# ipilter/RayTracerTest

Hardware: AMD Instinct MI355X
Metric: Mray/s at 1920x1080x16spp (higher is better)
Workload: dtype f32

## Files before the change

### include/rt_mi355x.h

```cpp
#ifndef RT_MI355X_H
#define RT_MI355X_H

#include <stddef.h>
#include <stdint.h>

#ifdef __cplusplus
extern "C" {
#endif

#define RT_OK              0
#define RT_ERR_INVALID     1
#define RT_ERR_NO_DEVICE   2
#define RT_ERR_HIP         3
#define RT_ERR_STATE       4

#define RT_MATH_FMA        0u
#define RT_MATH_STRICT     1u

#define RT_FLAG_NO_FILTER  1u
#define RT_FLAG_NO_BINNING 2u

#define RT_FLAG_NEAREST_HIT 4u

#define RT_FLAG_NO_MACRO_BINS 16u
// ... 153 lines not shown
int  rt_tracer_set_band(rt_tracer* t, uint32_t row_begin, uint32_t rows);
int  rt_tracer_gather_time(rt_tracer* t, double* total_ms, uint64_t* gathers, int reset_after);
int  rt_tracer_gather_only(rt_tracer* t);
int  rt_tracer_group_info(rt_tracer* t, char* json, size_t capacity);
int  rt_tracer_band_count(rt_tracer* t);
int  rt_tracer_band_info(rt_tracer* t, uint32_t band, uint32_t out[4]);

int rt_dbg_hit_triangle(int device, uint32_t math_mode, uint32_t n, const float* rays,
                        const float* tris, int eps_mode, int32_t* hit, float* tuv, float* normal,
                        float* point);
int rt_dbg_sincos(int device, uint32_t n, const float* x, float* s, float* c);
int rt_dbg_trace_occupancy(int device, int samples_in_flight, uint32_t lds_bytes);
int rt_dbg_valu_peak(int device, double* lane_fma_per_s, double* clock_ghz);
int rt_dbg_check_midrange(int device, uint64_t out[4]);
int rt_dbg_wave_list_counts(rt_tracer* t, int half, uint32_t* dst, size_t capacity_tiles, uint32_t* n_tiles, uint32_t* capacity_per_tile);
int rt_dbg_read_tile_lists(rt_tracer* t, uint32_t* dst, size_t capacity_words, uint32_t* words_per_tile);
int rt_dbg_focal_boxes(rt_tracer* t, float curv_scale, float* boxes, size_t boxes_capacity, float* focal, size_t focal_capacity);
int rt_dbg_classify(rt_tracer* t, uint32_t level, uint32_t forms, uint32_t slack_milli, const uint32_t* regions, uint32_t n_regions,
                    float* out, size_t capacity_floats);
int rt_dbg_bvh_build(const rt_float4* rows, size_t count, int edges_layout, void* nodes, size_t node_capacity_bytes,
                     void* leaf_records, size_t leaf_capacity_bytes, uint64_t info[8]);
int rt_dbg_feature_normals(const rt_float4* rows, size_t count, int edges_layout, void* out, size_t capacity_bytes, uint64_t info[8]);
int rt_dbg_exposure_rays(rt_tracer* t, const float* points, size_t n, const float* dirs, uint32_t n_dirs, uint32_t flags,
                         float* segs_out);
int rt_dbg_bvh_refit(const rt_float4* rows, size_t count, int edges_layout, void* nodes, size_t node_bytes, void* leaf_records,
                     size_t record_bytes, uint64_t info[8]);
double rt_dbg_bvh_tree_cost(const void* nodes, size_t node_bytes);
int rt_dbg_query_tree_read(rt_tracer* t, void* nodes, size_t node_capacity_bytes, void* records, size_t record_capacity_bytes,
                           uint64_t info[8]);
int rt_dbg_query_accel_slack(rt_tracer* t, uint32_t slack_milli);
int rt_dbg_query_stack_cap(rt_tracer* t, uint32_t cap);
int rt_dbg_uniform(int device, uint32_t n, uint32_t m, uint32_t* states, float* out);
int rt_dbg_get_ray(rt_tracer* t, uint32_t n, const uint32_t* pixels, uint32_t* states, float* rays);
void rt_dbg_rng_init_host(uint64_t seed, uint64_t subsequence, uint32_t state[6]);
void rt_dbg_rng_advance_host(uint32_t state[5], uint32_t n, int use_table);
void rt_dbg_rng_advance_host_n(uint32_t* states, uint32_t count, uint32_t n, int use_table);
int rt_dbg_owed_state(rt_tracer* t, uint64_t out[4]);
int rt_dbg_enqueue_calls(rt_tracer* t, uint64_t out[8]);

#ifdef __cplusplus
}
#endif
#endif
```

### raytracertest_amd/api.py

```python
import ctypes as C
import os
import threading
import weakref

import numpy as np

_HERE = os.path.dirname(os.path.abspath(__file__))
_LIB_PATH = os.environ.get("RT_MI355X_LIB") or os.path.join(_HERE, "lib", "librt_mi355x.so")

MATH_FMA, MATH_STRICT = 0, 1
FLAG_NO_FILTER = 1
FLAG_NO_BINNING = 2
FLAG_NEAREST_HIT = 4
FLAG_SMOOTH_NORMALS = 8
FLAG_NO_MACRO_BINS = 16
FLAG_NO_SUPER_BINS = 64
FLAG_NO_SURE_HIT = 32
BUF_RENDER, BUF_COUNTS, BUF_IMAGE, BUF_RNG, BUF_FRAME = 0, 1, 2, 3, 4
GROUP_ID_BYTES = 128
TRANSPORT_RCCL, TRANSPORT_PEER = 0, 1

ABI_SYMBOLS = [
    "rt_tracer_create", "rt_tracer_create_ex", "rt_tracer_destroy", "rt_tracer_trace",
    "rt_tracer_stop", "rt_tracer_resize", "rt_tracer_set_camera_parameters",
    "rt_tracer_rotate_camera", "rt_tracer_upload_scene", "rt_tracer_set_update_callback",
    "rt_tracer_set_finished_callback", "rt_tracer_wait", "rt_tracer_set_seed",
    "rt_tracer_upload_spheres", "rt_tracer_trace_enqueue", "rt_tracer_trace_enqueue_n", "rt_tracer_sync", "rt_tracer_trace_stats", "rt_tracer_launch", "rt_tracer_launch_iterations", "rt_tracer_fused_iterations", "rt_tracer_set_image_mirror", "rt_tracer_set_list_reuse", "rt_tracer_stream_b", "rt_tracer_upload_scene_edges", "rt_pack_normal",
    "rt_unpack_normal",
    "rt_tracer_kernel_time", "rt_tracer_launch_time", "rt_tracer_read_buffer", "rt_tracer_copy_buffer_to_device", "rt_tracer_copy_buffer_to_device_async",
    "rt_tracer_stream",
    "rt_tracer_device_pointer", "rt_tracer_buffer_bytes", "rt_tracer_info",
    "rt_tracer_last_error", "rt_last_error", "rt_device_count", "rt_version",
    "rt_dbg_hit_triangle", "rt_dbg_sincos", "rt_dbg_valu_peak", "rt_dbg_check_midrange", "rt_dbg_trace_occupancy", "rt_dbg_uniform", "rt_dbg_get_ray",
    "rt_dbg_rng_init_host", "rt_dbg_rng_advance_host", "rt_dbg_rng_advance_host_n", "rt_dbg_owed_state", "rt_dbg_enqueue_calls",
    "rt_tracer_create_multi", "rt_group_unique_id", "rt_tracer_join_group", "rt_tracer_leave_group",
    "rt_tracer_gather_time", "rt_tracer_band_count", "rt_tracer_band_info",
    "rt_tracer_join_group_bands", "rt_balance_rows", "rt_tracer_rebalance", "rt_tracer_set_band", "rt_dbg_read_tile_lists", "rt_dbg_wave_list_counts", "rt_dbg_focal_boxes", "rt_dbg_classify",
    "rt_tracer_gather_only", "rt_tracer_group_info",
    "rt_tracer_intersect", "rt_tracer_intersect_device", "rt_tracer_pick", "rt_tracer_focus_at",
    "rt_tracer_occluded", "rt_tracer_occluded_device",
    "rt_tracer_exposure", "rt_tracer_exposure_device", "rt_dbg_exposure_rays",
    "rt_tracer_intersect_all", "rt_tracer_intersect_all_device",
    "rt_tracer_closest_point", "rt_tracer_closest_point_device",
    "rt_tracer_closest_all", "rt_tracer_closest_all_device",
    "rt_tracer_signed_distance", "rt_tracer_signed_distance_device",
    "rt_tracer_closest_sides", "rt_tracer_closest_sides_device", "rt_dbg_feature_normals",
    "rt_tracer_overlap", "rt_tracer_overlap_device",
    "rt_tracer_set_query_accel", "rt_tracer_query_accel_info", "rt_dbg_bvh_build", "rt_dbg_query_accel_slack",
    "rt_tracer_set_query_accel_update", "rt_tracer_query_accel_rebuild", "rt_tracer_query_accel_update_info",
    "rt_dbg_bvh_refit", "rt_dbg_query_tree_read", "rt_dbg_bvh_tree_cost", "rt_dbg_query_stack_cap",
]


class RtError(RuntimeError):
    pass


PRIM_NONE = -1
RT_MAX_HITS = 16
RT_MAX_DIRS = 64
EXPOSURE_LOCAL, EXPOSURE_WORLD = 0, 1
QUERY_SCAN, QUERY_BVH = 0, 1
ACCEL_REBUILD, ACCEL_REFIT = 0, 1
BVH_NODE_DTYPE = np.dtype([("lo", np.float32, (3, 4)), ("hi", np.float32, (3, 4)), ("child", np.uint32, 4), ("cmax", np.float32, 4)])
BVH_RECORD_DTYPE = np.dtype([("e2", np.float32, 3), ("e1", np.float32, 3), ("v0", np.float32, 3), ("index", np.uint32), ("pad", np.uint32, 2)])
BVH_EMPTY, BVH_LEAF = 0xFFFFFFFF, 0x80000000
_ACCEL_KEYS = ("mode", "valid", "nodes", "leaves", "depth", "always_tested", "build_us", "device_bytes")
# ... 185 lines not shown
        L.rt_tracer_copy_buffer_to_device.argtypes = [vp, C.c_int, vp, C.c_size_t]
        L.rt_tracer_copy_buffer_to_device_async.argtypes = [vp, C.c_int, vp, C.c_size_t]
        L.rt_tracer_stream.argtypes = [vp]
        L.rt_tracer_stream.restype = vp
        L.rt_tracer_stream_b.argtypes = [vp]
        L.rt_tracer_stream_b.restype = vp
        L.rt_tracer_device_pointer.argtypes = [vp, C.c_int]
        L.rt_tracer_device_pointer.restype = vp
        L.rt_tracer_buffer_bytes.argtypes = [vp, C.c_int]
        L.rt_tracer_buffer_bytes.restype = C.c_size_t
        L.rt_tracer_info.argtypes = [vp, u32p]
        L.rt_tracer_last_error.argtypes = [vp]
        L.rt_tracer_last_error.restype = C.c_char_p
        L.rt_last_error.restype = C.c_char_p
        L.rt_device_count.restype = C.c_int
        L.rt_version.restype = C.c_char_p
        L.rt_dbg_hit_triangle.argtypes = [C.c_int, C.c_uint32, C.c_uint32, f32p, f32p, C.c_int,
                                          C.POINTER(C.c_int32), f32p, f32p, f32p]
        L.rt_dbg_sincos.argtypes = [C.c_int, C.c_uint32, f32p, f32p, f32p]
        L.rt_dbg_uniform.argtypes = [C.c_int, C.c_uint32, C.c_uint32, u32p, f32p]
        L.rt_dbg_valu_peak.argtypes = [C.c_int, C.POINTER(C.c_double), C.POINTER(C.c_double)]
        L.rt_dbg_trace_occupancy.argtypes = [C.c_int, C.c_int, C.c_uint32]
        L.rt_dbg_get_ray.argtypes = [vp, C.c_uint32, u32p, u32p, f32p]
        L.rt_dbg_rng_init_host.argtypes = [C.c_uint64, C.c_uint64, u32p]
        L.rt_dbg_rng_init_host.restype = None
        if hasattr(L, "rt_dbg_owed_state"):
            L.rt_dbg_rng_advance_host.argtypes = [u32p, C.c_uint32, C.c_int]
            L.rt_dbg_rng_advance_host.restype = None
            L.rt_dbg_rng_advance_host_n.argtypes = [u32p, C.c_uint32, C.c_uint32, C.c_int]
            L.rt_dbg_rng_advance_host_n.restype = None
            L.rt_dbg_owed_state.argtypes = [vp, C.POINTER(C.c_uint64)]
        if hasattr(L, "rt_dbg_enqueue_calls"):
            L.rt_dbg_enqueue_calls.argtypes = [vp, C.POINTER(C.c_uint64)]
        L.rt_tracer_create_multi.argtypes = [u32p, f32p, f32p, C.c_float, C.c_float, C.c_float, C.POINTER(Options),
                                             C.POINTER(C.c_int32), C.c_uint32, C.POINTER(vp)]
        L.rt_group_unique_id.argtypes = [C.c_char_p]
        L.rt_tracer_join_group.argtypes = [vp, C.c_uint32, C.c_uint32, C.c_char_p]
        L.rt_tracer_leave_group.argtypes = [vp]
        L.rt_tracer_gather_time.argtypes = [vp, C.POINTER(C.c_double), C.POINTER(C.c_uint64), C.c_int]
        L.rt_tracer_band_count.argtypes = [vp]
        L.rt_tracer_band_info.argtypes = [vp, C.c_uint32, u32p]
        L.rt_tracer_join_group_bands.argtypes = [vp, C.c_uint32, C.c_uint32, C.c_char_p, u32p]
        L.rt_balance_rows.argtypes = [C.c_uint32, u32p, C.POINTER(C.c_double), C.c_uint32, u32p]
        L.rt_tracer_rebalance.argtypes = [vp]
        L.rt_tracer_set_band.argtypes = [vp, C.c_uint32, C.c_uint32]
        L.rt_dbg_read_tile_lists.argtypes = [vp, u32p, C.c_size_t, u32p]
        L.rt_dbg_wave_list_counts.argtypes = [vp, C.c_int, u32p, C.c_size_t, u32p, u32p]
        L.rt_dbg_focal_boxes.argtypes = [vp, C.c_float, f32p, C.c_size_t, f32p, C.c_size_t]
        L.rt_tracer_gather_only.argtypes = [vp]
        L.rt_tracer_group_info.argtypes = [vp, C.c_char_p, C.c_size_t]
        L.rt_dbg_classify.argtypes = [vp, C.c_uint32, C.c_uint32, C.c_uint32, u32p, C.c_uint32, f32p, C.c_size_t]
        L.rt_tracer_intersect.argtypes = [vp, vp, C.c_size_t, vp]
        L.rt_tracer_intersect_device.argtypes = [vp, vp, C.c_size_t, vp, vp]
        L.rt_tracer_pick.argtypes = [vp, vp, C.c_size_t, vp, vp]
        L.rt_tracer_focus_at.argtypes = [vp, C.c_uint32, C.c_uint32, f32p]
        L.rt_tracer_occluded.argtypes = [vp, vp, C.c_size_t, vp]
        L.rt_tracer_occluded_device.argtypes = [vp, vp, C.c_size_t, vp, vp]
        L.rt_tracer_exposure.argtypes = [vp, vp, C.c_size_t, vp, C.c_uint32, C.c_uint32, vp]
        L.rt_tracer_exposure_device.argtypes = [vp, vp, C.c_size_t, vp, C.c_uint32, C.c_uint32, vp, vp]
        L.rt_dbg_exposure_rays.argtypes = [vp, vp, C.c_size_t, vp, C.c_uint32, C.c_uint32, vp]
        L.rt_tracer_intersect_all.argtypes = [vp, vp, C.c_size_t, C.c_uint32, vp, vp]
        L.rt_tracer_intersect_all_device.argtypes = [vp, vp, C.c_size_t, C.c_uint32, vp, vp, vp]
        L.rt_tracer_closest_point.argtypes = [vp, vp, C.c_size_t, vp]
        L.rt_tracer_closest_point_device.argtypes = [vp, vp, C.c_size_t, vp, vp]
        L.rt_tracer_closest_all.argtypes = [vp, vp, vp, C.c_size_t, C.c_uint32, vp, vp]
        L.rt_tracer_closest_all_device.argtypes = [vp, vp, vp, C.c_size_t, C.c_uint32, vp, vp, vp]
# ... 877 lines not shown
        raise RtError("rt_dbg_sincos failed (%d): %s" % (rc, L.rt_last_error().decode()))
    return s, c


def dbg_valu_peak(device=0):
    L = load_library()
    r, g = C.c_double(), C.c_double()
    rc = L.rt_dbg_valu_peak(device, C.byref(r), C.byref(g))
    if rc != 0:
        raise RtError("rt_dbg_valu_peak failed (%d): %s" % (rc, L.rt_last_error().decode()))
    return r.value, g.value


def dbg_check_midrange(device=0):
    L = load_library()
    out = (C.c_uint64 * 4)()
    L.rt_dbg_check_midrange.argtypes = [C.c_int, C.POINTER(C.c_uint64)]
    rc = L.rt_dbg_check_midrange(device, out)
    if rc != 0:
        raise RtError("rt_dbg_check_midrange failed (%d): %s" % (rc, L.rt_last_error().decode()))
    return tuple(int(x) for x in out)


def dbg_uniform(states, m, device=0):
    L = load_library()
    st = np.ascontiguousarray(states, np.uint32).reshape(-1, 6).copy()
    out = np.zeros((st.shape[0], m), np.float32)
    rc = L.rt_dbg_uniform(device, st.shape[0], m, _u32p(st), _f32p(out))
    if rc != 0:
        raise RtError("rt_dbg_uniform failed (%d): %s" % (rc, L.rt_last_error().decode()))
    return out, st


def dbg_rng_init_host(seed, subsequence):
    s = np.zeros(6, np.uint32)
    load_library().rt_dbg_rng_init_host(int(seed), int(subsequence), _u32p(s))
    return s


def dbg_rng_advance_host(state, n, use_table):
    s = np.ascontiguousarray(state, np.uint32).copy()
    L = load_library()
    if s.ndim == 1:
        L.rt_dbg_rng_advance_host(_u32p(s.reshape(5)), int(n), int(bool(use_table)))
    else:
        L.rt_dbg_rng_advance_host_n(_u32p(s.reshape(-1, 5)), s.reshape(-1, 5).shape[0], int(n), int(bool(use_table)))
    return s
```

### raytracertest_amd/csrc/rt_debug.hip

```cpp
#include "rt_tracer.hpp"

using namespace rtr;

template <class F>
static int on_device(int device, F&& f) {
  const int rc = require_device(device);
  if (rc != RT_OK) return rc;
  return guarded(nullptr, [&] { HIP_CHECK(hipSetDevice(device)); f(); });
}

template <class F>
static int on_tracer(rt_tracer* t, F&& f) { return exclusive(t, [&] { t->use_device(); f(); }); }

extern "C" {

int rt_dbg_hit_triangle(int device, uint32_t math_mode, uint32_t n, const float* rays, const float* tris,
                        int eps_mode, int32_t* hit, float* tuv, float* normal, float* point) {
  return on_device(device, [&] {
    DevArray<float> dr(n * 6), dt(n * 9), duv(n * 3), dn(n * 3), dp(n * 3);
    DevArray<int> dh(n);
    HIP_CHECK(hipMemcpy(dr.get(), rays, n * 6 * sizeof(float), hipMemcpyHostToDevice));
    HIP_CHECK(hipMemcpy(dt.get(), tris, n * 9 * sizeof(float), hipMemcpyHostToDevice));
    HIP_CHECK(rtk::launch_dbg_hit_triangle(math_mode != RT_MATH_STRICT, n, dr.get(), dt.get(), eps_mode, dh.get(), duv.get(),
                                           dn.get(), dp.get(), nullptr));
// ... 136 lines not shown
    const size_t tiles = static_cast<size_t>((t->W + 31u) / 32u) * ((t->rows + 7u) / 8u) * 4u;
    const size_t nb = tiles * 8u, nf = static_cast<size_t>(t->npix()) * 3u;
    if (nb > boxes_capacity || nf > focal_capacity) throw HipFail{fmt("focal boxes need %zu + %zu floats", nb, nf)};
    DevArray<float> db(nb), df(nf);
    HIP_CHECK(hipMemsetAsync(db.get(), 0, nb * sizeof(float), t->main_stream()));
    HIP_CHECK(rtk::launch_dbg_focal_boxes(t->fma, p, db.get(), df.get(), t->main_stream()));
    HIP_CHECK(hipStreamSynchronize(t->main_stream()));
    HIP_CHECK(hipMemcpy(boxes, db.get(), nb * sizeof(float), hipMemcpyDeviceToHost));
    HIP_CHECK(hipMemcpy(focal, df.get(), nf * sizeof(float), hipMemcpyDeviceToHost));
  });
}

int rt_dbg_classify(rt_tracer* t, uint32_t level, uint32_t forms, uint32_t slack_milli, const uint32_t* regions, uint32_t n_regions,
                    float* out, size_t capacity_floats) {
  if (!t || t->mg || !regions || !out || level > 4u) return RT_ERR_INVALID;
  return on_tracer(t, [&] {
    rtk::TraceParams p = t->params(1);
    p.macro_w = rt_tracer::kMacroW; p.macro_h = rt_tracer::kMacroH;
    p.super_f = rt_tracer::kSuperF;
    const uint32_t rw = level == 0u ? 8u : level == 2u ? p.macro_w : level == 4u ? p.macro_w * p.super_f : 32u;
    const uint32_t rh = level == 2u ? p.macro_h : level == 4u ? p.macro_h * p.super_f : level == 3u ? 16u : 8u;
    for (uint32_t i = 0; i < n_regions; ++i)
      if (regions[2u * i] % rw != 0u || regions[2u * i + 1u] % rh != 0u || regions[2u * i] >= t->W || regions[2u * i + 1u] >= t->rows)
        throw HipFail{fmt("region %u (%u, %u) is not a level-%u region of the %ux%u band", i, regions[2u * i], regions[2u * i + 1u], level, t->W, t->rows)};
    const size_t per = 16u + static_cast<size_t>(t->n_tris) * (forms ? 32u : 12u);
    if (per * n_regions > capacity_floats) throw HipFail{fmt("rt_dbg_classify needs %zu floats", per * n_regions)};
    DevArray<uint32_t> dr(static_cast<size_t>(n_regions) * 2u);
    DevArray<float> dout(per * n_regions);
    HIP_CHECK(hipMemcpyAsync(dr.get(), regions, static_cast<size_t>(n_regions) * 2u * sizeof(uint32_t), hipMemcpyHostToDevice, t->main_stream()));
    HIP_CHECK(rtk::launch_dbg_classify(t->fma, forms != 0u, slack_milli, p, level, n_regions, dr.get(), dout.get(), t->main_stream()));
    HIP_CHECK(hipStreamSynchronize(t->main_stream()));
    HIP_CHECK(hipMemcpy(out, dout.get(), per * n_regions * sizeof(float), hipMemcpyDeviceToHost));
  });
}

void rt_dbg_rng_init_host(uint64_t seed, uint64_t subsequence, uint32_t state[6]) {
  rth::init_state(jump_host(), seed, subsequence & 0xffffffffull, state);
}


void rt_dbg_rng_advance_host_n(uint32_t* states, uint32_t count, uint32_t n, int use_table) {
  if (use_table) {
    const std::vector<uint32_t> table = rth::build_window_table(rth::step_power(n));
    for (uint32_t i = 0; i < count; ++i) rth::window_product(table, states + 5u * i, states + 5u * i);
    return;
  }
  constexpr uint32_t kLanes = 64;
  for (uint32_t base = 0; base < count; base += kLanes) {
    const uint32_t m = count - base < kLanes ? count - base : kLanes;
    uint32_t v[5][kLanes] = {};
    for (uint32_t i = 0; i < m; ++i) for (int w = 0; w < 5; ++w) v[w][i] = states[5u * (base + i) + w];
    auto f = [](uint32_t x, uint32_t y) -> uint32_t { const uint32_t t = x ^ (x >> 2); return (y ^ (y << 4)) ^ (t ^ (t << 1)); };
    uint32_t k = 0;
    for (; k + 5u <= n; k += 5u)
      for (uint32_t i = 0; i < kLanes; ++i) {
        v[0][i] = f(v[0][i], v[4][i]); v[1][i] = f(v[1][i], v[0][i]); v[2][i] = f(v[2][i], v[1][i]);
        v[3][i] = f(v[3][i], v[2][i]); v[4][i] = f(v[4][i], v[3][i]);
      }
    for (uint32_t i = 0; i < m; ++i) {
      uint32_t one[5] = {v[0][i], v[1][i], v[2][i], v[3][i], v[4][i]};
      for (uint32_t r = k; r < n; ++r) rth::xorshift_step(one);
      memcpy(states + 5u * (base + i), one, sizeof one);
    }
  }
}
void rt_dbg_rng_advance_host(uint32_t state[5], uint32_t n, int use_table) { rt_dbg_rng_advance_host_n(state, 1u, n, use_table); }
// ... 20 lines not shown
```

### raytracertest_amd/csrc/rt_device_math.hpp

```cpp
#pragma once
#include <hip/hip_runtime.h>
#include <stdint.h>

namespace rtd {

struct V3 { float x, y, z; };

__device__ __forceinline__ V3 sub(V3 a, V3 b) { return {a.x - b.x, a.y - b.y, a.z - b.z}; }
__device__ __forceinline__ V3 add(V3 a, V3 b) { return {a.x + b.x, a.y + b.y, a.z + b.z}; }
__device__ __forceinline__ float absf(float f) { return (f < 0.0f) ? -f : f; }

__device__ __forceinline__ bool midrange(float x) {
  return (__builtin_bit_cast(uint32_t, x) - 0x0F800000u) <= (0x6F800000u - 0x0F800000u);
}
__device__ __forceinline__ float sqrt_midrange(float x) {
  const float s = __builtin_amdgcn_sqrtf(x);
  const float s_dn = __builtin_bit_cast(float, __builtin_bit_cast(int, s) - 1);
  const float s_up = __builtin_bit_cast(float, __builtin_bit_cast(int, s) + 1);
  const float r_dn = __builtin_fmaf(-s_dn, s, x);
  const float r_up = __builtin_fmaf(-s_up, s, x);
  float r = (r_dn <= 0.0f) ? s_dn : s;
  r = (r_up > 0.0f) ? s_up : r;
  return r;
}
// ... 27 lines not shown
  static __device__ __forceinline__ float dot(V3 a, V3 b) {
    if constexpr (FMA) return __builtin_fmaf(a.z, b.z, __builtin_fmaf(a.x, b.x, a.y * b.y));
    else return ((a.x * b.x) + (a.y * b.y)) + (a.z * b.z);
  }
  static __device__ __forceinline__ V3 normalize(V3 a) {
    const float dd = dot(a, a);
    float inv;
#ifndef RT_NO_MIDRANGE
    if (__builtin_amdgcn_ballot_w64(!midrange(dd)) == 0ull) inv = rcp_midrange(sqrt_midrange(dd));
    else
#endif
      inv = 1.0f / __builtin_sqrtf(dd);
    return {a.x * inv, a.y * inv, a.z * inv};
  }
  static __device__ __forceinline__ V3 mat_mul_point(const float* M, float x, float y, float z, float w) {
    return {madd2(M[0], x, M[3], y) + madd2(M[6], z, M[9], w),
            madd2(M[1], x, M[4], y) + madd2(M[7], z, M[10], w),
            madd2(M[2], x, M[5], y) + madd2(M[8], z, M[11], w)};
  }
};

__host__ __device__ __forceinline__ void sincos_spec(float x, float& s, float& c) {
  const float k = __builtin_rintf(x * 0.63661977236758134308f);
  float r = __builtin_fmaf(k, -1.5703125f, x);
  r = __builtin_fmaf(k, -4.837512969970703125e-4f, r);
  r = __builtin_fmaf(k, -7.54978995489188216e-8f, r);
  const float z = r * r;
  const float ps = __builtin_fmaf(__builtin_fmaf(-1.9515295891e-4f, z, 8.3321608736e-3f), z,
                                  -1.6666654611e-1f);
  const float sn = __builtin_fmaf(r * z, ps, r);
  const float pc = __builtin_fmaf(__builtin_fmaf(2.443315711809948e-5f, z, -1.388731625493765e-3f), z,
                                  4.166664568298827e-2f);
  const float cs = __builtin_fmaf(z * z, pc, __builtin_fmaf(-0.5f, z, 1.0f));
  const int q = static_cast<int>(k) & 3;
  const float ss = (q & 1) ? cs : sn;
  const float cc = (q & 1) ? sn : cs;
  s = (q & 2) ? -ss : ss;
  c = ((q + 1) & 2) ? -cc : cc;
}

struct Rng { uint32_t d, v0, v1, v2, v3, v4; };

__device__ __forceinline__ uint32_t rng_next(Rng& s) {
  const uint32_t t = s.v0 ^ (s.v0 >> 2);
  s.v0 = s.v1; s.v1 = s.v2; s.v2 = s.v3; s.v3 = s.v4;
  s.v4 = (s.v4 ^ (s.v4 << 4)) ^ (t ^ (t << 1));
  s.d += 362437u;
  return s.v4 + s.d;
}

__device__ __forceinline__ void rng_discard(Rng& s, uint32_t draws) {
  auto f = [](uint32_t x, uint32_t v) -> uint32_t { const uint32_t t = x ^ (x >> 2); return (v ^ (v << 4)) ^ (t ^ (t << 1)); };
  uint32_t i = 0;
  for (; i + 5u <= draws; i += 5u) {
    s.v0 = f(s.v0, s.v4); s.v1 = f(s.v1, s.v0); s.v2 = f(s.v2, s.v1); s.v3 = f(s.v3, s.v2); s.v4 = f(s.v4, s.v3);
  }
  for (; i < draws; ++i) {
    const uint32_t nv = f(s.v0, s.v4);
    s.v0 = s.v1; s.v1 = s.v2; s.v2 = s.v3; s.v3 = s.v4; s.v4 = nv;
  }
  s.d += 362437u * draws;
}

__device__ __forceinline__ float rng_uniform(Rng& s) {
  return __builtin_fmaf(static_cast<float>(rng_next(s)), 2.3283064e-10f, 2.3283064e-10f / 2.0f);
}

__device__ __forceinline__ void uniform_on_disk(Rng& s, float& dx, float& dy) {
  const float t = (2.0f * 3.14156545f) * rng_uniform(s);
  const float u1 = rng_uniform(s);
  const float u2 = rng_uniform(s);
// ... 28 lines not shown
```

### raytracertest_amd/csrc/rt_kernels.hpp

```cpp
#pragma once
#include <hip/hip_runtime.h>
#include <hip/hip_ext.h>
#include <stdint.h>
#include <atomic>

namespace rtk {

constexpr uint32_t kSuperChunk = 1024u, kSuperMaxChunks = 64u;

struct TraceParams {
  float4*   render;
  uint32_t* rng;
  uint32_t  weyl, count;
  uint32_t  W, H;
  uint32_t  row0, rows;
  uint32_t  npix;
  uint32_t  samples;
  float     cam[12];
  float     half_height, aspect, focal, aperture;
  float     tile_curv, tile_round;
  const float4* tri_a;
  const float*  tri_b;
  const float4* tri_color;
  uint32_t  n_tris;
  const float4* spheres;
  uint32_t  n_spheres;
  uint32_t  chunk;
  uint32_t  bin_list;
  uint32_t  block_list;
  unsigned long long* stats;
  uint32_t* image;
  const float4* tri_n;
#ifdef RT_TIMELINE
  unsigned long long* timeline;
#endif
  uint32_t* image_host;
  uint32_t  pretest_on;
  uint32_t  iters;
  uint32_t* macro_lists;
  uint32_t  macro_cap, macro_w, macro_h, macro_nx;
  uint32_t* super_lists;
  uint32_t  super_chunks, super_f, super_nx;
  float*    macro_bounds;
  uint32_t* tile_lists;
  uint32_t  row_il, row_phase;
  uint32_t* half_cost;
  uint32_t  cost_split_brow;
  const float4* sure_table;
  uint32_t* wave_lists;
  uint32_t  wave_cap;
  uint32_t  flags;
};

constexpr uint32_t TRACE_ZERO_ACC = 1u;
constexpr uint32_t TRACE_EMIT_IMAGE = 2u;
constexpr uint32_t TRACE_NEAREST_HIT = 4u;
constexpr uint32_t TRACE_PRETEST = 32u;
constexpr uint32_t TRACE_NO_SURE_HIT = 64u;
constexpr uint32_t TRACE_OWE_RNG = 128u;

enum class TracePath : uint32_t {
  FullScan,
  SmallLists,
  Classify,
  ClassifyForms,
  DenseLists,
};

constexpr uint64_t kRngInitMaxPixels = (1ull << 32) - (1ull << 19);
hipError_t launch_rng_init(uint32_t* rng, uint32_t npix, uint32_t p0, const uint32_t seeded[6],
                           const uint32_t* jump, const uint32_t* win, hipStream_t st);
hipError_t launch_rng_settle(const TraceParams& p, uint32_t draws, const uint32_t* table, hipStream_t st);
hipError_t launch_prep_triangles(bool fma, bool edges, const float4* verts, uint32_t n, float4* tri_a, float* tri_b,
                                 float4* color, float4* normals, hipStream_t st);
uint32_t trace_lds_bytes(const TraceParams& p, TracePath path);
inline dim3 trace_grid(const TraceParams& p) {
  dim3 grid((p.W + 31u) / 32u, (p.rows + 7u) / 8u);
  if (p.row_il != 0u) {
    const uint32_t R = grid.y, G = p.row_il, full = R / (2u * G), rest = R % (2u * G);
    grid.y = full * G + (p.row_phase == 0u ? (rest < G ? rest : G) : (rest > G ? rest - G : 0u));
  }
  return grid;
}
struct KernelTable {
  std::atomic<hipFunction_t> trace[2][3][2][5][2][2] = {};
  std::atomic<hipFunction_t> lists[2][4] = {};
};
hipError_t launch_trace(const TraceParams& p, bool fma, bool filter, TracePath path, int K, hipStream_t st, KernelTable* table = nullptr,
                        hipEvent_t stop = nullptr);
int trace_occupancy(int K, size_t lds);
hipError_t launch_convert(const float4* render, uint32_t count, uint32_t* image, uint32_t npix, hipStream_t st);

// ... 69 lines not shown
```

### raytracertest_amd/csrc/rt_rays.hpp

```cpp
#pragma once
#include <float.h>
#include <type_traits>

#include "rt_device_math.hpp"
#include "rt_kernels.hpp"

namespace rtk {

using rtd::Math;
using rtd::Rng;
using rtd::V3;

#define RT_EPS 0.0000000001f

template <bool FMA>
__device__ __forceinline__ bool hit_triangle_exact(V3 o, V3 d, V3 v0, V3 e1, V3 e2, float eps,
                                                   float& t, float& u, float& v, int& stage) {
  using M = Math<FMA>;
  stage = 0;
  const V3 pv = M::cross(d, e2);
  const float det = M::dot(e1, pv);
  if (det < eps) return false;
  stage = 1;
  const float inv = 1.0f / det;
// ... 18 lines not shown
  const float dvv = M::dot(vv, vv);
  float cc, disc;
  if constexpr (FMA) {
    cc = __builtin_fmaf(-sph.w, sph.w, dvv);
    disc = __builtin_fmaf(b, b, -((4.0f * a) * cc));
  } else {
    cc = dvv - sph.w * sph.w;
    disc = b * b - (4.0f * a) * cc;
  }
  if (disc < 0.0f) return false;
  t = (-b - __builtin_sqrtf(disc)) / (2.0f * a);
  return true;
}

template <bool FMA>
__device__ __forceinline__ void pinhole(const TraceParams& p, uint32_t px, uint32_t py, V3& o, V3& d) {
  using M = Math<FMA>;
  const float nx = (static_cast<float>(px) + 0.5f) / static_cast<float>(p.W);
  const float ny = (static_cast<float>(py) + 0.5f) / static_cast<float>(p.H);
  const float cx = ((2.0f * nx - 1.0f) * p.half_height) * p.aspect;
  const float cy = (1.0f - 2.0f * ny) * p.half_height;
  o = M::mat_mul_point(p.cam, 0.0f, 0.0f, 0.0f, 1.0f);
  const V3 pw = M::mat_mul_point(p.cam, cx, cy, -1.0f, 1.0f);
  d = M::normalize(rtd::sub(pw, o));
}

template <bool FMA>
__device__ __forceinline__ V3 focal_point(const TraceParams& p, V3 pd) {
  using M = Math<FMA>;
  return {M::madd1(p.focal, pd.x, p.cam[9]), M::madd1(p.focal, pd.y, p.cam[10]),
          M::madd1(p.focal, pd.z, p.cam[11])};
}

template <bool FMA>
__device__ __forceinline__ void get_ray(const TraceParams& p, V3 focal, Rng& rng, V3& o, V3& d) {
  using M = Math<FMA>;
  float dx, dy;
  rtd::uniform_on_disk(rng, dx, dy);
  const V3 pos = {p.cam[9], p.cam[10], p.cam[11]};
  const V3 off = {dx * p.aperture, dy * p.aperture, 0.0f};
  o = rtd::add(pos, off);
  d = M::normalize(rtd::sub(focal, o));
}


}
```

### raytracertest_amd/csrc/rt_trace.hpp

```cpp
#pragma once
#include "rt_lists.hpp"

namespace rtk {


template <bool FMA, int K, bool FILTER, bool STATS, class GetB>
__device__ __forceinline__ void test_triangle(const float4 A0, const float4 A1, GetB get_v0z, int tri_index,
                                              const V3 (&o)[K], const V3 (&d)[K], float (&best_t)[K],
                                              int (&best_i)[K], bool nearest, bool counted_lane, uint32_t valid_k,
                                              unsigned long long (&st_exit)[4],
                                              unsigned long long (&st_skip)[4]) {
  using M = Math<FMA>;
  const V3 e2 = {A0.x, A0.y, A0.z}, e1 = {A0.w, A1.x, A1.y};

  if constexpr (!FILTER) {
    const V3 v0 = {A1.z, A1.w, get_v0z()};
#pragma unroll
    for (int k = 0; k < K; ++k) {
      float t = 0.0f, u = 0.0f, v = 0.0f;
      int stage;
      const bool h = hit_triangle_exact<FMA>(o[k], d[k], v0, e1, e2, RT_EPS, t, u, v, stage);
      if (h && (nearest ? (t > 0.0f && t < best_t[k]) : best_t[k] < t)) {
        best_t[k] = t;
        best_i[k] = tri_index;
// ... 18 lines not shown
      live |= mk[k];
    }
    if (live == 0ull) { if constexpr (STATS) st_skip[0]++; return; }

    const V3 v0 = {A1.z, A1.w, get_v0z()};
    V3 tv[K];
    float U[K], thi[K], tlo[K];
    live = 0ull;
#pragma unroll
    for (int k = 0; k < K; ++k) {
      tv[k] = rtd::sub(o[k], v0);
      U[k] = M::dot(tv[k], pv[k]);
      thi[k] = det[k] * 1.0001f;
      tlo[k] = det[k] * -1e-6f;
      mk[k] &= __builtin_amdgcn_ballot_w64(!(U[k] > thi[k])) & __builtin_amdgcn_ballot_w64(!(U[k] < tlo[k]));
      live |= mk[k];
    }
    if (live == 0ull) { if constexpr (STATS) st_skip[1]++; return; }

    V3 qv[K];
    float V[K];
    live = 0ull;
#pragma unroll
    for (int k = 0; k < K; ++k) {
      qv[k] = M::cross(tv[k], e1);
      V[k] = M::dot(d[k], qv[k]);
      mk[k] &= __builtin_amdgcn_ballot_w64(!(V[k] < tlo[k])) &
               __builtin_amdgcn_ballot_w64(!((U[k] + V[k]) > thi[k]));
      live |= mk[k];
    }
    if (live == 0ull) { if constexpr (STATS) st_skip[2]++; return; }
    if constexpr (STATS) st_skip[3]++;

#pragma unroll
    for (int k = 0; k < K; ++k) {
      if (mk[k] != 0ull) {
        const float inv = 1.0f / det[k];
        const float u = U[k] * inv;
        const float v = V[k] * inv;
        const float t = M::dot(e2, qv[k]) * inv;
        const bool miss = (det[k] < RT_EPS) | (u < 0.0f) | (u > 1.0f) | (v < 0.0f) | (u + v > 1.0f);
        const bool closer = nearest ? ((t > 0.0f) & (t < best_t[k])) : (best_t[k] < t);
        const bool upd = (!miss) & closer;
        best_t[k] = upd ? t : best_t[k];
        best_i[k] = upd ? tri_index : best_i[k];
      }
    }
  }
}


constexpr uint32_t kWaveRec = 16u;
constexpr uint32_t kWaveOverflow = 0xFFFFFFFFu;
template <bool FMA, int K, bool FILTER, bool STATS, TracePath Path, bool FUSE = false>
__global__ __launch_bounds__(256, (Path == TracePath::SmallLists && K == 2) ? 5 : 4) void trace_kernel(const TraceParams p) {
  static_assert(Path != TracePath::DenseLists || (FILTER && !STATS), "lists from HBM: the default dense-scene kernels only");
  using M = Math<FMA>;
  extern __shared__ float4 s_mem[];
  const uint32_t lane = threadIdx.x & 63u;
  const uint32_t wave = threadIdx.x >> 6;
  const uint32_t bx = blockIdx.x;
  uint32_t by = blockIdx.y;
  const uint32_t gxb = gridDim.x;
  if constexpr (Path == TracePath::SmallLists) {
    if (p.row_il != 0u) by = (blockIdx.y / p.row_il) * (2u * p.row_il) + p.row_phase * p.row_il + blockIdx.y % p.row_il;
  }
  const uint32_t px = bx * 32u + wave * 8u + (lane & 7u);
  const uint32_t ly = by * 8u + (lane >> 3);
  const bool inside = px < p.W && ly < p.rows;
  const uint32_t cxp = inside ? px : 0u, cyp = inside ? ly : 0u;
// ... 241 lines not shown
      for (uint32_t base = 0; base < (sure_hit_tile ? 0u : count); base += 64u) {
        const uint32_t e = base + lane;
        if (e < count) {
          const uint32_t tri = saved[1u + e];
          cA[2u * e] = p.tri_a[2u * tri];
          cA[2u * e + 1u] = p.tri_a[2u * tri + 1u];
          cB[e] = p.tri_b[tri];
          cI[e] = static_cast<int>(tri);
        }
      }
    }
    __builtin_amdgcn_fence(__ATOMIC_RELEASE, "wavefront");
    __builtin_amdgcn_wave_barrier();
    list_count = count;
    if constexpr (STATS) { st_bin[0] += count; st_bin[1] += 1; }
    list_complete = true;
  }
  bool forms_ready = false;
  if constexpr (Path == TracePath::ClassifyForms) {
    const uint32_t next0 = classify(0u, std::true_type{});
    list_complete = next0 >= src_count;
    forms_ready = pretest && list_complete;
  }
  if constexpr (Path == TracePath::DenseLists) forms_ready = true;
  if constexpr (RNG_LATE) load_rng();
  tl_mark(1);
  float4 sure_col = make_float4(0.0f, 0.0f, 0.0f, 0.0f);
  const bool sure_sums = Path == TracePath::SmallLists && p.sure_table != nullptr;
  if constexpr (Path == TracePath::SmallLists) { if (sure_hit_tile) sure_col = sure_sums ? p.sure_table[sure_winner] : p.tri_color[sure_winner]; }
  if constexpr (STATS && Path == TracePath::SmallLists) {
    if (lane == 0u && p.stats != nullptr)
      atomicAdd(p.stats + (sure_hit_tile ? 13 : list_count == 0u ? 11 : list_count == 1u ? 12 : list_count == 2u ? 14 : 15), 1ull);
  }
  const uint32_t iters = FUSE ? p.iters : 1u;
  float rx = 0.0f, ry = 0.0f, rz = 0.0f, rw = 0.0f;
  for (uint32_t it = 0; it < iters; ++it) {
  if constexpr (FUSE) { ax = 0.0f; ay = 0.0f; az = 0.0f; }
  uint32_t traced_samples = p.samples;
  if constexpr (Path == TracePath::SmallLists) {
    if (sure_hit_tile) {
      if (!owes_rng) rtd::rng_discard(rng, 3u * p.samples);
      if (sure_sums) { ax = sure_col.x; ay = sure_col.y; az = sure_col.z; }
      else for (uint32_t s = 0; s < p.samples; ++s) { ax += sure_col.x; ay += sure_col.y; az += sure_col.z; }
      if constexpr (STATS) st_pre += (p.samples + static_cast<uint32_t>(K) - 1u) / static_cast<uint32_t>(K);
      traced_samples = 0u;
    }
  }
  for (uint32_t s0 = 0; s0 < traced_samples; s0 += K) {
    if (s0 == static_cast<uint32_t>(K)) tl_mark(2);
    const uint32_t valid_k = (p.samples - s0 < static_cast<uint32_t>(K)) ? p.samples - s0 : static_cast<uint32_t>(K);
    V3 o[K], d[K];
    float best_t[K];
    int best_i[K];
#pragma unroll
    for (int k = 0; k < K; ++k) {
      if (static_cast<uint32_t>(k) < valid_k) get_ray<FMA>(p, focal, rng, o[k], d[k]);
      else { o[k] = {0.0f, 0.0f, 0.0f}; d[k] = {0.0f, 0.0f, -1.0f}; }
      best_t[k] = nearest ? FLT_MAX : -FLT_MAX;
      best_i[k] = -1;
    }

    const unsigned long long lanes_in = __builtin_amdgcn_ballot_w64(inside);
    unsigned long long pad_mask[K];
#pragma unroll
    for (int k = 0; k < K; ++k) pad_mask[k] = (static_cast<uint32_t>(k) < valid_k) ? 0ull : ~0ull;
    float dox[K], doy[K];
    float dFx = 0.0f, dFy = 0.0f, dFz = 0.0f;
    if constexpr (PRETEST) {
#pragma unroll
      for (int k = 0; k < K; ++k) { dox[k] = o[k].x - p.cam[9]; doy[k] = o[k].y - p.cam[10]; }
      dFx = focal.x - fam.fc[0]; dFy = focal.y - fam.fc[1]; dFz = focal.z - fam.fc[2];
    }
    if constexpr (Path == TracePath::SmallLists) {
      for (uint32_t j = 0; j < list_count; ++j) {
        const float4 A0 = cA[2u * j], A1 = cA[2u * j + 1u];
        test_triangle<FMA, K, FILTER, STATS>(A0, A1, [&] { return cB[j]; }, cI[j], o, d, best_t, best_i,
                                             nearest, inside, valid_k, st_exit, st_skip);
      }
// ... 98 lines not shown
              const float4 A0 = p.tri_a[2 * win], A1 = p.tri_a[2 * win + 1];
              float t = 0.0f, u = 0.0f, v = 0.0f;
              int stage;
              (void)hit_triangle_exact<FMA>(o[k], d[k], {A1.z, A1.w, p.tri_b[win]}, {A0.w, A1.x, A1.y},
                                            {A0.x, A0.y, A0.z}, RT_EPS, t, u, v, stage);
              const float4 n0 = p.tri_n[3 * win], n1 = p.tri_n[3 * win + 1], n2 = p.tri_n[3 * win + 2];
              const float w = (1.0f - u) - v;
              V3 m;
              if constexpr (FMA) {
                m.x = __builtin_fmaf(v, n2.x, __builtin_fmaf(u, n1.x, w * n0.x));
                m.y = __builtin_fmaf(v, n2.y, __builtin_fmaf(u, n1.y, w * n0.y));
                m.z = __builtin_fmaf(v, n2.z, __builtin_fmaf(u, n1.z, w * n0.z));
              } else {
                m.x = (w * n0.x + u * n1.x) + v * n2.x;
                m.y = (w * n0.y + u * n1.y) + v * n2.y;
                m.z = (w * n0.z + u * n1.z) + v * n2.z;
              }
              const V3 nn = M::normalize(m);
              r = rtd::absf(nn.x); g = rtd::absf(nn.y); b = rtd::absf(nn.z);
            } else if (by_slot) {
              r = cC[3 * win]; g = cC[3 * win + 1]; b = cC[3 * win + 2];
            } else {
              const float4 col = p.tri_color[win];
              r = col.x; g = col.y; b = col.z;
            }
          } else {
            const float4 sph = p.spheres[win - first_sphere];
            const V3 hp = {M::madd1(d[k].x, dist, o[k].x), M::madd1(d[k].y, dist, o[k].y),
                           M::madd1(d[k].z, dist, o[k].z)};
            const V3 nn = M::normalize(rtd::sub(hp, {sph.x, sph.y, sph.z}));
            r = rtd::absf(nn.x); g = rtd::absf(nn.y); b = rtd::absf(nn.z);
          }
        } else {
          if constexpr (FMA) {
            r = __builtin_fmaf(d[k].x, 0.2f, 0.15f * 0.8f);
            g = __builtin_fmaf(d[k].y, 0.2f, 0.11f * 0.8f);
            b = __builtin_fmaf(d[k].z, 0.2f, 0.13f * 0.8f);
          } else {
            r = 0.15f * 0.8f + d[k].x * 0.2f;
            g = 0.11f * 0.8f + d[k].y * 0.2f;
            b = 0.13f * 0.8f + d[k].z * 0.2f;
          }
        }
        ax += r; ay += g; az += b;
      }
    }
  }

  if constexpr (FUSE) {
    if (it == 0u && !(p.flags & TRACE_ZERO_ACC) && inside) {
      const float4 r0 = p.render[pix];
      rx = r0.x; ry = r0.y; rz = r0.z; rw = r0.w;
    }
    rx += ax; ry += ay; rz += az;
  }
  }
  tl_mark(3);
  uint32_t pix_lo = static_cast<uint32_t>(pix);
  asm volatile("" : "+v"(pix_lo));
  const size_t pix_e = pix_lo;
  if (inside) {
    float4 acc_in = make_float4(0.0f, 0.0f, 0.0f, 0.0f);
    if constexpr (!FUSE) {
      if (!(p.flags & TRACE_ZERO_ACC)) acc_in = p.render[pix_e];
    }
    const uint32_t cnt = p.count + iters * p.samples;
    float4 acc = acc_in;
    if constexpr (FUSE) {
      acc = make_float4(rx, ry, rz, rw);
    } else {
      acc.x += ax; acc.y += ay; acc.z += az;
    }
    p.render[pix_e] = acc;
    if (p.flags & TRACE_EMIT_IMAGE) {
      const float c = static_cast<float>(cnt);
// ... 32 lines not shown
```

### raytracertest_amd/csrc/rt_tracer.hpp

```cpp
#pragma once
#include <algorithm>
#include <atomic>
#include <chrono>
#include <condition_variable>
#include <functional>
#include <map>
#include <cmath>
#include <cstdio>
#include <cstring>
#include <ctime>
#include <mutex>
#include <optional>
#include <string>
#include <thread>
#include <vector>

#include "../../include/rt_mi355x.h"
#include "rt_device_math.hpp"
#include "rt_hip_host.hpp"
#include "rt_kernels.hpp"
#include "rt_query_state.hpp"
#include "rt_rng_host.hpp"

namespace rtr {
// ... 615 lines not shown
    HIP_CHECK(hipMemcpyAsync(target, d_image.get(), static_cast<size_t>(npix()) * sizeof(uint32_t), hipMemcpyDeviceToDevice, main_stream()));
  }

  void tile_corner_bound(rtk::TraceParams& p) const {
    p.tile_curv = -1.0f; p.tile_round = 0.0f;
    double G[3][3];
    for (int i = 0; i < 3; ++i)
      for (int j = 0; j < 3; ++j) {
        G[i][j] = 0.0;
        for (int r = 0; r < 3; ++r) G[i][j] += static_cast<double>(p.cam[i * 3 + r]) * static_cast<double>(p.cam[j * 3 + r]);
      }
    double lmax = 0.0, lmin = 1e300;
    for (int i = 0; i < 3; ++i) {
      const double off = std::fabs(G[i][(i + 1) % 3]) + std::fabs(G[i][(i + 2) % 3]);
      lmax = std::max(lmax, G[i][i] + off);
      lmin = std::min(lmin, G[i][i] - off);
    }
    if (!(lmin > 0.25) || !(lmax < 4.0)) return;
    const double hh = std::fabs(static_cast<double>(p.half_height)), asp = std::fabs(static_cast<double>(p.aspect));
    const double a = 7.0 * 2.0 * hh * asp / static_cast<double>(W), b = 7.0 * 2.0 * hh / static_cast<double>(H);
    if (!(0.5 * (a * a + b * b) * (lmax / lmin) <= 0.1 * std::min(a, b))) return;
    const double foc = std::fabs(static_cast<double>(p.focal));
#ifndef RT_TILE_CURV_SCALE
#define RT_TILE_CURV_SCALE 1.0
#endif
    const double curv = foc * 0.5 * (a * a + b * b) * (lmax / lmin) * 1.001 * RT_TILE_CURV_SCALE + 1e-30;
    const double pos = std::max(std::fabs(p.cam[9]), std::max(std::fabs(p.cam[10]), std::fabs(p.cam[11])));
    const double round = foc * (1.0 + hh * asp + hh) + pos;
    if (!(curv <= 1e30) || !(round <= 1e30)) return;
    p.tile_curv = std::nextafter(static_cast<float>(curv), 3.0e38f);
    p.tile_round = std::nextafter(static_cast<float>(round), 3.0e38f);
  }

  rtk::TraceParams params(uint32_t samples) {
    rtk::TraceParams p;
    memset(&p, 0, sizeof p);
    rtr::Camera c;
    { std::lock_guard<std::mutex> lk(state_mu); c = cam; }
    p.render = d_render.get(); p.rng = d_rng.get();
    p.W = W; p.H = H; p.row0 = row0; p.rows = rows; p.npix = npix(); p.samples = samples;
    for (int col = 0; col < 4; ++col)
      for (int r = 0; r < 3; ++r) p.cam[col * 3 + r] = c.M[col * 4 + r];
    p.half_height = c.tan_half_fov();
    p.aspect = static_cast<float>(W) / static_cast<float>(H);
    p.focal = c.focal; p.aperture = c.aperture;
    tile_corner_bound(p);
    p.tri_a = d_tri.get(); p.tri_b = d_tri_b.get(); p.tri_color = d_tri_color.get(); p.n_tris = n_tris;
    p.tri_n = smooth_normals ? d_tri_n.get() : nullptr;
    p.stats = nullptr;
    p.spheres = d_spheres.get(); p.n_spheres = n_spheres;
    p.chunk = chunk_req ? chunk_req : 1024u;
    if (p.chunk > 4096u) p.chunk = 4096u;
    uint32_t want = bin_list_req ? bin_list_req : ((n_tris + 31u) / 32u) * 32u;
    want = ((want + 31u) / 32u) * 32u;
    p.bin_list = want < 32u ? 32u : want > (bin_list_req ? 960u : 256u) ? (bin_list_req ? 960u : 256u) : want;
    p.block_list = n_tris > p.bin_list ? 1024u : 0u;
    if (p.block_list != 0u && !bin_list_req) p.bin_list = 192u;
    if (pretest && filter && bin && n_tris >= kPretestMinTris && n_tris <= 50000u) {
      p.pretest_on = 1u;
      if (!bin_list_req) p.bin_list = RT_PRETEST_LIST;
      else p.bin_list = (p.bin_list + 1u) & ~1u;
      if (p.block_list != 0u) p.block_list = 448u;
    }
    return p;
  }

  uint32_t mode_flags(const rtk::TraceParams& p) const {
    return (nearest_hit ? rtk::TRACE_NEAREST_HIT : 0u) | (p.pretest_on ? rtk::TRACE_PRETEST : 0u) |
           (sure_hit ? 0u : rtk::TRACE_NO_SURE_HIT);
  }

  int pick_k(uint32_t samples) const {
    if (k_req == 1 || k_req == 2 || k_req == 4) return static_cast<int>(k_req);
    const uint32_t want = (n_tris <= 128u) ? 2u : 4u;
    return samples >= want ? static_cast<int>(want) : samples >= 2 ? 2 : 1;
  }

  void enqueue_trace_launch(uint32_t samples, uint32_t flags, int sync_after, uint32_t iters = 1,
                            uint32_t* host_image = nullptr, bool allow_split = true) {
    const int K = pick_k(samples);
    rtk::TraceParams p = params(samples);
    p.iters = iters;
    p.image_host = host_image;
    p.flags = flags | mode_flags(p);
    p.image = d_image.get();
    const rtk::TracePath path = trace_path(p);
    std::unique_lock<std::recursive_mutex> uniform_lk(order_mu);
    const std::optional<rtr::OweKey> okey = owe_key_of(p, path);
    const bool owes = debt.owes(okey);
    if (!owes) settle();
    debt.key = okey;
    bool have_lists = false;
    const bool build_lists = prepare_tile_lists(p, path, (flags & rtk::TRACE_ZERO_ACC) != 0u, have_lists);
    attach_sure_table(p, have_lists);
    if (owes) p.flags |= rtk::TRACE_OWE_RNG;
    last_k = K; last_chunk = p.chunk;
    last_lds = rtk::trace_lds_bytes(p, path == rtk::TracePath::DenseLists ? rtk::TracePath::ClassifyForms : path);
    const uint32_t r0 = allow_split ? split_row(p.rows) : 0u;
    rtr::EventPair e;
    const bool timed = clock.start(sync_after == 1, r0 != 0u, e);
    words.take(p);
    if (owes) debt.add(p);
// ... 325 lines not shown
```

Measured before the change: 677,500.

## Add fast background-only tile path and midrange reciprocal paths for rays and hits

Adds a host-side check that bounds the camera basis, position, focal distance and aperture, and sets a flag when every ray direction length is guaranteed midrange. When the flag is set, tiles with empty triangle lists and no spheres, smooth normals or nearest-hit mode skip the full tracing loop and only generate rays to shade the background. Ray normalization uses cheap midrange sqrt and rcp in that case. Separately, triangle hit inversion uses a midrange reciprocal when the whole wave's determinants are bounded, and the sincos sign selection becomes bit XORs. Risks are small numeric differences from approximate reciprocals and extra ballot work per hit batch.

```diff
diff --git a/include/rt_mi355x.h b/include/rt_mi355x.h
--- a/include/rt_mi355x.h
+++ b/include/rt_mi355x.h
@@ -209,6 +209,7 @@
 int rt_dbg_query_stack_cap(rt_tracer* t, uint32_t cap);
 int rt_dbg_uniform(int device, uint32_t n, uint32_t m, uint32_t* states, float* out);
 int rt_dbg_get_ray(rt_tracer* t, uint32_t n, const uint32_t* pixels, uint32_t* states, float* rays);
+int rt_dbg_direction_range(const float cam[12], float half_height, float aspect, float focal, float aperture);
 void rt_dbg_rng_init_host(uint64_t seed, uint64_t subsequence, uint32_t state[6]);
 void rt_dbg_rng_advance_host(uint32_t state[5], uint32_t n, int use_table);
 void rt_dbg_rng_advance_host_n(uint32_t* states, uint32_t count, uint32_t n, int use_table);
diff --git a/raytracertest_amd/api.py b/raytracertest_amd/api.py
--- a/raytracertest_amd/api.py
+++ b/raytracertest_amd/api.py
@@ -32,7 +32,7 @@
     "rt_tracer_device_pointer", "rt_tracer_buffer_bytes", "rt_tracer_info",
     "rt_tracer_last_error", "rt_last_error", "rt_device_count", "rt_version",
     "rt_dbg_hit_triangle", "rt_dbg_sincos", "rt_dbg_valu_peak", "rt_dbg_check_midrange", "rt_dbg_trace_occupancy", "rt_dbg_uniform", "rt_dbg_get_ray",
-    "rt_dbg_rng_init_host", "rt_dbg_rng_advance_host", "rt_dbg_rng_advance_host_n", "rt_dbg_owed_state", "rt_dbg_enqueue_calls",
+    "rt_dbg_direction_range", "rt_dbg_rng_init_host", "rt_dbg_rng_advance_host", "rt_dbg_rng_advance_host_n", "rt_dbg_owed_state", "rt_dbg_enqueue_calls",
     "rt_tracer_create_multi", "rt_group_unique_id", "rt_tracer_join_group", "rt_tracer_leave_group",
     "rt_tracer_gather_time", "rt_tracer_band_count", "rt_tracer_band_info",
     "rt_tracer_join_group_bands", "rt_balance_rows", "rt_tracer_rebalance", "rt_tracer_set_band", "rt_dbg_read_tile_lists", "rt_dbg_wave_list_counts", "rt_dbg_focal_boxes", "rt_dbg_classify",
@@ -284,6 +284,8 @@
             L.rt_dbg_owed_state.argtypes = [vp, C.POINTER(C.c_uint64)]
         if hasattr(L, "rt_dbg_enqueue_calls"):
             L.rt_dbg_enqueue_calls.argtypes = [vp, C.POINTER(C.c_uint64)]
+        if hasattr(L, "rt_dbg_direction_range"):
+            L.rt_dbg_direction_range.argtypes = [f32p, C.c_float, C.c_float, C.c_float, C.c_float]
         L.rt_tracer_create_multi.argtypes = [u32p, f32p, f32p, C.c_float, C.c_float, C.c_float, C.POINTER(Options),
                                              C.POINTER(C.c_int32), C.c_uint32, C.POINTER(vp)]
         L.rt_group_unique_id.argtypes = [C.c_char_p]
@@ -1227,6 +1229,11 @@
     return out, st
 
 
+def dbg_direction_range(cam, half_height, aspect, focal, aperture):
+    c = np.ascontiguousarray(cam, np.float32).reshape(12)
+    return bool(load_library().rt_dbg_direction_range(_f32p(c), float(half_height), float(aspect), float(focal), float(aperture)))
+
+
 def dbg_rng_init_host(seed, subsequence):
     s = np.zeros(6, np.uint32)
     load_library().rt_dbg_rng_init_host(int(seed), int(subsequence), _u32p(s))
diff --git a/raytracertest_amd/csrc/rt_debug.hip b/raytracertest_amd/csrc/rt_debug.hip
--- a/raytracertest_amd/csrc/rt_debug.hip
+++ b/raytracertest_amd/csrc/rt_debug.hip
@@ -192,6 +192,10 @@
     HIP_CHECK(hipStreamSynchronize(t->main_stream()));
     HIP_CHECK(hipMemcpy(out, dout.get(), per * n_regions * sizeof(float), hipMemcpyDeviceToHost));
   });
+}
+
+int rt_dbg_direction_range(const float cam[12], float half_height, float aspect, float focal, float aperture) {
+  return (cam != nullptr && rt_tracer::direction_range_vouched(cam, half_height, aspect, focal, aperture)) ? 1 : 0;
 }
 
 void rt_dbg_rng_init_host(uint64_t seed, uint64_t subsequence, uint32_t state[6]) {
diff --git a/raytracertest_amd/csrc/rt_device_math.hpp b/raytracertest_amd/csrc/rt_device_math.hpp
--- a/raytracertest_amd/csrc/rt_device_math.hpp
+++ b/raytracertest_amd/csrc/rt_device_math.hpp
@@ -83,11 +83,11 @@
   const float pc = __builtin_fmaf(__builtin_fmaf(2.443315711809948e-5f, z, -1.388731625493765e-3f), z,
                                   4.166664568298827e-2f);
   const float cs = __builtin_fmaf(z * z, pc, __builtin_fmaf(-0.5f, z, 1.0f));
-  const int q = static_cast<int>(k) & 3;
-  const float ss = (q & 1) ? cs : sn;
-  const float cc = (q & 1) ? sn : cs;
-  s = (q & 2) ? -ss : ss;
-  c = ((q + 1) & 2) ? -cc : cc;
+  const uint32_t q = static_cast<uint32_t>(static_cast<int>(k));
+  const float ss = (q & 1u) ? cs : sn;
+  const float cc = (q & 1u) ? sn : cs;
+  s = __builtin_bit_cast(float, __builtin_bit_cast(uint32_t, ss) ^ ((q << 30) & 0x80000000u));
+  c = __builtin_bit_cast(float, __builtin_bit_cast(uint32_t, cc) ^ (((q + 1u) << 30) & 0x80000000u));
 }
 
 struct Rng { uint32_t d, v0, v1, v2, v3, v4; };
diff --git a/raytracertest_amd/csrc/rt_kernels.hpp b/raytracertest_amd/csrc/rt_kernels.hpp
--- a/raytracertest_amd/csrc/rt_kernels.hpp
+++ b/raytracertest_amd/csrc/rt_kernels.hpp
@@ -19,6 +19,7 @@
   float     cam[12];
   float     half_height, aspect, focal, aperture;
   float     tile_curv, tile_round;
+  uint32_t  dir_vouched;
   const float4* tri_a;
   const float*  tri_b;
   const float4* tri_color;
@@ -58,6 +59,7 @@
 constexpr uint32_t TRACE_PRETEST = 32u;
 constexpr uint32_t TRACE_NO_SURE_HIT = 64u;
 constexpr uint32_t TRACE_OWE_RNG = 128u;
+constexpr uint32_t TRACE_DIR_MIDRANGE = 256u;
 
 enum class TracePath : uint32_t {
   FullScan,
diff --git a/raytracertest_amd/csrc/rt_rays.hpp b/raytracertest_amd/csrc/rt_rays.hpp
--- a/raytracertest_amd/csrc/rt_rays.hpp
+++ b/raytracertest_amd/csrc/rt_rays.hpp
@@ -74,7 +74,7 @@
           M::madd1(p.focal, pd.z, p.cam[11])};
 }
 
-template <bool FMA>
+template <bool FMA, bool VOUCHED = false>
 __device__ __forceinline__ void get_ray(const TraceParams& p, V3 focal, Rng& rng, V3& o, V3& d) {
   using M = Math<FMA>;
   float dx, dy;
@@ -82,7 +82,37 @@
   const V3 pos = {p.cam[9], p.cam[10], p.cam[11]};
   const V3 off = {dx * p.aperture, dy * p.aperture, 0.0f};
   o = rtd::add(pos, off);
-  d = M::normalize(rtd::sub(focal, o));
+  if constexpr (VOUCHED) {
+    const V3 a = rtd::sub(focal, o);
+    const float inv = rtd::rcp_midrange(rtd::sqrt_midrange(M::dot(a, a)));
+    d = {a.x * inv, a.y * inv, a.z * inv};
+  } else {
+    d = M::normalize(rtd::sub(focal, o));
+  }
+}
+
+template <bool FMA>
+__device__ __forceinline__ V3 background(V3 d) {
+  if constexpr (FMA) return {__builtin_fmaf(d.x, 0.2f, 0.15f * 0.8f), __builtin_fmaf(d.y, 0.2f, 0.11f * 0.8f), __builtin_fmaf(d.z, 0.2f, 0.13f * 0.8f)};
+  else return {0.15f * 0.8f + d.x * 0.2f, 0.11f * 0.8f + d.y * 0.2f, 0.13f * 0.8f + d.z * 0.2f};
+}
+
+template <bool FMA, int K>
+__device__ __forceinline__ void background_samples(const TraceParams& p, V3 focal, Rng& rng, float& ax, float& ay, float& az) {
+  uint32_t s = 0;
+  for (; s + static_cast<uint32_t>(K) <= p.samples; s += static_cast<uint32_t>(K)) {
+    V3 o[K], d[K];
+#pragma unroll
+    for (int k = 0; k < K; ++k) get_ray<FMA, true>(p, focal, rng, o[k], d[k]);
+#pragma unroll
+    for (int k = 0; k < K; ++k) { const V3 c = background<FMA>(d[k]); ax += c.x; ay += c.y; az += c.z; }
+  }
+  for (; s < p.samples; ++s) {
+    V3 o, d;
+    get_ray<FMA, true>(p, focal, rng, o, d);
+    const V3 c = background<FMA>(d);
+    ax += c.x; ay += c.y; az += c.z;
+  }
 }
 
 
diff --git a/raytracertest_amd/csrc/rt_trace.hpp b/raytracertest_amd/csrc/rt_trace.hpp
--- a/raytracertest_amd/csrc/rt_trace.hpp
+++ b/raytracertest_amd/csrc/rt_trace.hpp
@@ -74,10 +74,14 @@
     if (live == 0ull) { if constexpr (STATS) st_skip[2]++; return; }
     if constexpr (STATS) st_skip[3]++;
 
+    unsigned long long wide = 0ull;
+#pragma unroll
+    for (int k = 0; k < K; ++k) wide |= __builtin_amdgcn_ballot_w64(!(det[k] <= 0x1p96f));
+    const bool det_midrange = wide == 0ull;
 #pragma unroll
     for (int k = 0; k < K; ++k) {
       if (mk[k] != 0ull) {
-        const float inv = 1.0f / det[k];
+        const float inv = det_midrange ? rtd::rcp_midrange(det[k]) : 1.0f / det[k];
         const float u = U[k] * inv;
         const float v = V[k] * inv;
         const float t = M::dot(e2, qv[k]) * inv;
@@ -385,6 +389,8 @@
     if (lane == 0u && p.stats != nullptr)
       atomicAdd(p.stats + (sure_hit_tile ? 13 : list_count == 0u ? 11 : list_count == 1u ? 12 : list_count == 2u ? 14 : 15), 1ull);
   }
+  const bool dir_vouched = Path == TracePath::SmallLists && (p.flags & TRACE_DIR_MIDRANGE) != 0u;
+  const bool background_tile = dir_vouched && !sure_hit_tile && list_count == 0u && p.n_spheres == 0u && p.tri_n == nullptr && !nearest;
   const uint32_t iters = FUSE ? p.iters : 1u;
   float rx = 0.0f, ry = 0.0f, rz = 0.0f, rw = 0.0f;
   for (uint32_t it = 0; it < iters; ++it) {
@@ -397,6 +403,12 @@
       else for (uint32_t s = 0; s < p.samples; ++s) { ax += sure_col.x; ay += sure_col.y; az += sure_col.z; }
       if constexpr (STATS) st_pre += (p.samples + static_cast<uint32_t>(K) - 1u) / static_cast<uint32_t>(K);
       traced_samples = 0u;
+    }
+    if constexpr (!STATS) {
+      if (background_tile) {
+        background_samples<FMA, K>(p, focal, rng, ax, ay, az);
+        traced_samples = 0u;
+      }
     }
   }
   for (uint32_t s0 = 0; s0 < traced_samples; s0 += K) {
@@ -561,15 +573,8 @@
             r = rtd::absf(nn.x); g = rtd::absf(nn.y); b = rtd::absf(nn.z);
           }
         } else {
-          if constexpr (FMA) {
-            r = __builtin_fmaf(d[k].x, 0.2f, 0.15f * 0.8f);
-            g = __builtin_fmaf(d[k].y, 0.2f, 0.11f * 0.8f);
-            b = __builtin_fmaf(d[k].z, 0.2f, 0.13f * 0.8f);
-          } else {
-            r = 0.15f * 0.8f + d[k].x * 0.2f;
-            g = 0.11f * 0.8f + d[k].y * 0.2f;
-            b = 0.13f * 0.8f + d[k].z * 0.2f;
-          }
+          const V3 c = background<FMA>(d[k]);
+          r = c.x; g = c.y; b = c.z;
         }
         ax += r; ay += g; az += b;
       }
diff --git a/raytracertest_amd/csrc/rt_tracer.hpp b/raytracertest_amd/csrc/rt_tracer.hpp
--- a/raytracertest_amd/csrc/rt_tracer.hpp
+++ b/raytracertest_amd/csrc/rt_tracer.hpp
@@ -671,6 +671,29 @@
     p.tile_round = std::nextafter(static_cast<float>(round), 3.0e38f);
   }
 
+  static bool direction_range_vouched(const float cam[12], float half_height, float aspect, float focal, float aperture) {
+    for (int i = 0; i < 3; ++i) {
+      double g[3];
+      for (int j = 0; j < 3; ++j) {
+        g[j] = 0.0;
+        for (int r = 0; r < 3; ++r) g[j] += static_cast<double>(cam[i * 3 + r]) * static_cast<double>(cam[j * 3 + r]);
+      }
+      const double off = std::fabs(g[(i + 1) % 3]) + std::fabs(g[(i + 2) % 3]);
+      if (!(g[i] - off > 0.25) || !(g[i] + off < 4.0)) return false;
+    }
+    const double hh = std::fabs(static_cast<double>(half_height)), asp = std::fabs(static_cast<double>(aspect));
+    double P = 0.0;
+    for (int i = 9; i < 12; ++i) {
+      if (!(std::fabs(static_cast<double>(cam[i])) <= 4096.0)) return false;
+      P = std::max(P, std::fabs(static_cast<double>(cam[i])));
+    }
+    if (!(hh * asp + hh + 1.0 <= 4096.0)) return false;
+    const double f = std::fabs(static_cast<double>(focal)), A = std::fabs(static_cast<double>(aperture));
+    const double E = (f + P + A) * 0x1p-20;
+    const double lo = f * (1.0 - 0x1p-20) - 1.01 * A - E, hi = f * (1.0 + 0x1p-20) + 1.01 * A + E;
+    return lo >= 0x1p-40 && hi <= 0x1p40;
+  }
+
   rtk::TraceParams params(uint32_t samples) {
     rtk::TraceParams p;
     memset(&p, 0, sizeof p);
@@ -684,6 +707,7 @@
     p.aspect = static_cast<float>(W) / static_cast<float>(H);
     p.focal = c.focal; p.aperture = c.aperture;
     tile_corner_bound(p);
+    p.dir_vouched = direction_range_vouched(p.cam, p.half_height, p.aspect, p.focal, p.aperture) ? 1u : 0u;
     p.tri_a = d_tri.get(); p.tri_b = d_tri_b.get(); p.tri_color = d_tri_color.get(); p.n_tris = n_tris;
     p.tri_n = smooth_normals ? d_tri_n.get() : nullptr;
     p.stats = nullptr;
@@ -706,7 +730,7 @@
 
   uint32_t mode_flags(const rtk::TraceParams& p) const {
     return (nearest_hit ? rtk::TRACE_NEAREST_HIT : 0u) | (p.pretest_on ? rtk::TRACE_PRETEST : 0u) |
-           (sure_hit ? 0u : rtk::TRACE_NO_SURE_HIT);
+           (sure_hit ? 0u : rtk::TRACE_NO_SURE_HIT) | (p.dir_vouched ? rtk::TRACE_DIR_MIDRANGE : 0u);
   }
 
   int pick_k(uint32_t samples) const {
```

Measured after the change: 671,500. Within noise of the previous version (-0.9%).
